# bioinformatics-centre/kaiju

Measured on NVIDIA H100. Metric: reads/sec (150 bp paired, MEM mode, synth-viruses .fmi), higher is better.
Workload: dtype int64

## Files before the change

### include/kaiju_b200.h

```cpp
#ifndef KAIJU_B200_H
#define KAIJU_B200_H
#include <stdint.h>

#ifdef __cplusplus
extern "C" {
#endif

typedef enum {
    KJ_OK = 0,
    KJ_ERR_ARG = -1,
    KJ_ERR_IO = -2,
    KJ_ERR_CUDA = -3,
    KJ_ERR_NO_DEVICE = -4,
    KJ_ERR_UNSUPPORTED = -5,
    KJ_ERR_OVERFLOW = -6,
    KJ_ERR_NOMEM = -7
} kj_status;

#define KJ_MAX_READ_LEN 16383
#define KJ_MAX_PROTEIN_LEN 5461
#define KJ_MAX_LONG_READ_LEN 1048575

typedef struct {
    int32_t mode;
// ... 102 lines not shown
    int32_t min_read_count;
    int32_t expand_viruses;
    int32_t filter_unclassified;
    int32_t full_path;
    const char *rank_list;
} kj_table_opts;
int kj_table_write(const uint64_t *taxon_ids, const uint64_t *counts, uint64_t n, const char *nodes_dmp, const char *names_dmp,
                   const char *label, const kj_table_opts *opts, const char *out_path, int append);
int kj_counts_table(kj_ctx *ctx, const char *nodes_dmp, const char *names_dmp, const char *label, const kj_table_opts *opts,
                    const char *out_path, int append);

int kj_check_errors(kj_ctx *ctx);

const char *kj_last_error(void);
uint64_t kj_kernel_launches(const kj_ctx *ctx);
uint64_t kj_index_bytes(const kj_ctx *ctx);
uint64_t kj_index_host_bytes(const kj_ctx *ctx);
int kj_index_layout(const kj_ctx *ctx);
double kj_last_kernel_ms(const kj_ctx *ctx);
int kj_launch_geometry(const kj_ctx *ctx, int *grid, int *block, int *dyn_smem_bytes);
int kj_version(void);
int kj_debug_index_checksums(kj_ctx *ctx, uint64_t out[8]);
int kj_debug_host_index_checksums(const kj_index_view *index, const kj_taxonomy_view *taxonomy, uint64_t out[8]);
int kj_debug_inflate_bgzf(kj_ctx *ctx, const uint8_t *file_bytes, uint64_t n, uint8_t *out, uint64_t out_cap, uint64_t *out_n,
                          uint64_t *first_bad_offset);

#ifdef __cplusplus
}
#endif
#endif
```

### kaiju_b200/__init__.py

```python
import ctypes as C
import os
import numpy as np

_HERE = os.path.dirname(os.path.abspath(__file__))
LIB_PATH = os.environ.get("KJ_B200_LIB") or os.path.join(_HERE, "libkaijub200.so")
MAX_READ_LEN = 16383
MAX_LONG_READ_LEN = 1048575

MEM, GREEDY = 0, 1
OUT_KAIJU, OUT_KAIJU_IDS, OUT_KAIJU_V, OUT_NAMES, OUT_NAMES_V = 0, 1, 2, 3, 4
STR_ACCESSION, STR_TAXON = 0, 1


class KjParams(C.Structure):
    _fields_ = [("mode", C.c_int32), ("min_fragment_length", C.c_uint32), ("mismatches", C.c_uint32),
                ("min_score", C.c_uint32), ("seed_length", C.c_uint32), ("use_evalue", C.c_int32),
                ("min_evalue", C.c_double), ("seg", C.c_int32), ("input_is_protein", C.c_int32), ("name_mode", C.c_int32)]


class KjIndexView(C.Structure):
    _fields_ = [("alen", C.c_int32), ("alphabet", C.c_char_p), ("bwtlen", C.c_int64), ("bwt", C.c_void_p),
                ("startLcode", C.c_void_p), ("db_len", C.c_int64), ("nseq", C.c_int32), ("ncheck", C.c_int64),
                ("chpt_exp", C.c_int32), ("nbytes", C.c_int32), ("pbits", C.c_int32), ("sa", C.c_void_p),
                ("seq_taxon", C.c_void_p), ("seq_accession", C.c_void_p)]
# ... 15 lines not shown
_lib = None


def lib():
    global _lib
    if _lib is None:
        if not os.path.exists(LIB_PATH):
            raise KaijuError("kaiju_b200: %s is missing -- build it with `make -C kaiju_b200/csrc` "
                             "(or python -c 'import __graft_entry__ as g; g.build()'). There is no CPU fallback." % LIB_PATH)
        L = C.CDLL(LIB_PATH)
        L.kj_last_error.restype = C.c_char_p
        L.kj_fmi_load.argtypes = [C.c_char_p, C.POINTER(C.c_void_p)]
        L.kj_fmi_view.argtypes = [C.c_void_p, C.POINTER(KjIndexView)]
        L.kj_fmi_free.argtypes = [C.c_void_p]
        L.kj_nodes_load.argtypes = [C.c_char_p, C.POINTER(C.c_void_p)]
        L.kj_nodes_view.argtypes = [C.c_void_p, C.POINTER(KjTaxonomyView)]
        L.kj_nodes_free.argtypes = [C.c_void_p]
        L.kj_create.argtypes = [C.POINTER(C.c_void_p), C.c_int, C.POINTER(KjParams), C.POINTER(KjIndexView), C.POINTER(KjTaxonomyView)]
        if hasattr(L, "kj_create_scaled"):
            L.kj_create_scaled.argtypes = [C.POINTER(C.c_void_p), C.c_int, C.POINTER(KjParams), C.POINTER(KjIndexView), C.POINTER(KjTaxonomyView), C.c_uint32]
            L.kj_index_build_ms.restype = C.c_double; L.kj_index_build_ms.argtypes = [C.c_void_p]
            L.kj_debug_index_checksums.argtypes = [C.c_void_p, C.c_void_p]
            L.kj_debug_host_index_checksums.argtypes = [C.POINTER(KjIndexView), C.POINTER(KjTaxonomyView), C.c_void_p]
            L.kj_classify_multi.argtypes = [C.POINTER(C.c_void_p), C.c_int, C.c_void_p, C.c_void_p, C.c_void_p, C.c_void_p, C.c_uint64, C.c_void_p, C.c_void_p]
            L.kj_device_count.restype = C.c_int
            L.kj_classify2.argtypes = [C.c_void_p, C.c_void_p, C.c_void_p, C.c_void_p, C.c_void_p, C.c_uint64, C.c_void_p, C.c_void_p, C.c_void_p]
            L.kj_classify_device2.argtypes = [C.c_void_p, C.c_void_p, C.c_void_p, C.c_void_p, C.c_void_p, C.c_uint64, C.c_uint32, C.c_uint32,
                                              C.c_void_p, C.c_void_p, C.c_void_p, C.c_void_p]
        L.kj_native_index_write.argtypes = [C.POINTER(KjIndexView), C.POINTER(KjTaxonomyView), C.c_char_p]
        L.kj_create_from_native.argtypes = [C.POINTER(C.c_void_p), C.c_int, C.POINTER(KjParams), C.c_char_p]
        L.kj_set_params.argtypes = [C.c_void_p, C.POINTER(KjParams)]
        L.kj_set_max_read_len.argtypes = [C.c_void_p, C.c_uint32]
        L.kj_destroy.argtypes = [C.c_void_p]
        L.kj_classify.argtypes = [C.c_void_p, C.c_void_p, C.c_void_p, C.c_void_p, C.c_void_p, C.c_uint64, C.c_void_p, C.c_void_p]
        L.kj_classify_verbose.argtypes = [C.c_void_p, C.c_void_p, C.c_void_p, C.c_void_p, C.c_void_p, C.c_uint64, C.c_void_p, C.c_void_p, C.c_void_p, C.c_void_p]
        L.kj_classify_device.argtypes = [C.c_void_p, C.c_void_p, C.c_void_p, C.c_void_p, C.c_void_p, C.c_uint64, C.c_uint32, C.c_uint32,
                                         C.c_void_p, C.c_void_p, C.c_void_p]
        L.kj_kernel_launches.restype = C.c_uint64; L.kj_kernel_launches.argtypes = [C.c_void_p]
        L.kj_index_bytes.restype = C.c_uint64; L.kj_index_bytes.argtypes = [C.c_void_p]
        if hasattr(L, "kj_create_tiered"):
            L.kj_create_tiered.argtypes = [C.POINTER(C.c_void_p), C.c_int, C.POINTER(KjParams), C.POINTER(KjIndexView), C.POINTER(KjTaxonomyView), C.c_uint32, C.c_uint64]
            L.kj_index_host_bytes.restype = C.c_uint64; L.kj_index_host_bytes.argtypes = [C.c_void_p]
        if hasattr(L, "kj_create_group"):
            L.kj_create_group.argtypes = [C.POINTER(C.c_void_p), C.c_int, C.POINTER(C.c_int), C.POINTER(KjParams), C.POINTER(KjIndexView), C.POINTER(KjTaxonomyView), C.c_uint32]
        if hasattr(L, "kj_index_layout"):
            L.kj_index_layout.restype = C.c_int; L.kj_index_layout.argtypes = [C.c_void_p]
# ... 291 lines not shown
    @property
    def kernel_launches(self):
        return int(lib().kj_kernel_launches(self._ctx))

    @property
    def index_bytes(self):
        return int(lib().kj_index_bytes(self._ctx))

    @property
    def layout(self):
        return int(lib().kj_index_layout(self._ctx))

    @property
    def host_bytes(self):
        return int(lib().kj_index_host_bytes(self._ctx))

    @property
    def index_build_ms(self):
        return float(lib().kj_index_build_ms(self._ctx))

    def debug_index_checksums(self):
        out = np.zeros(8, dtype=np.uint64); _check(lib().kj_debug_index_checksums(self._ctx, out.ctypes.data)); return out

    @property
    def last_kernel_ms(self):
        return float(lib().kj_last_kernel_ms(self._ctx))

    @property
    def launch_geometry(self):
        g = C.c_int(); b = C.c_int(); s = C.c_int()
        lib().kj_launch_geometry(self._ctx, C.byref(g), C.byref(b), C.byref(s))
        return g.value, b.value, s.value
```

### kaiju_b200/csrc/kj_build.h

```cpp
#pragma once

#define KJ_BLD_THREADS 256
struct KjBuildLcode { uint8_t v[256]; };

template <int RB>
__global__ void __launch_bounds__(KJ_BLD_THREADS) kj_bld_count(const uint8_t* __restrict__ bwt, const __grid_constant__ KjBuildLcode lc, uint64_t n, uint32_t rep, int alen,
                                                                uint32_t* __restrict__ tile_counts) {
    __shared__ uint32_t tot[KJ_MAX_ALEN];
    __shared__ uint8_t lcs[256];
    __shared__ uint8_t cnt[KJ_MAX_ALEN * KJ_BLD_THREADS];
    if (threadIdx.x < KJ_MAX_ALEN) tot[threadIdx.x] = 0;
    lcs[threadIdx.x] = lc.v[threadIdx.x];
    for (int a = 0; a < KJ_MAX_ALEN; a++) cnt[a * KJ_BLD_THREADS + threadIdx.x] = 0;
    __syncthreads();
    const uint64_t tile_rows = (uint64_t)KJ_BLD_THREADS * RB, start = (uint64_t)blockIdx.x * tile_rows;
    for (uint32_t i = threadIdx.x; i < tile_rows; i += KJ_BLD_THREADS) {
        const uint64_t row = start + i;
        if (row < n) cnt[(uint32_t)lcs[bwt[rep == 1 ? row : row / rep]] * KJ_BLD_THREADS + threadIdx.x]++;
    }
    for (int a = 0; a < alen; a++) {
        uint32_t v = cnt[a * KJ_BLD_THREADS + threadIdx.x];
        for (int m = 16; m > 0; m >>= 1) v += __shfl_xor_sync(0xffffffffu, v, m);
        if ((threadIdx.x & 31) == 0 && v) atomicAdd(&tot[a], v);
    }
// ... 74 lines not shown
        letters[wd] = v;
    }
}
__global__ void kj_bld_sa_tax(const uint8_t* __restrict__ sa, uint64_t n_entries, uint64_t first, int nbytes, int pbits, uint32_t nseq, const uint32_t* __restrict__ seq_tax,
                              uint32_t* __restrict__ sa_tax, uint32_t* __restrict__ err) {
    for (uint64_t e = (uint64_t)blockIdx.x * blockDim.x + threadIdx.x; e < n_entries; e += (uint64_t)gridDim.x * blockDim.x) {
        const uint8_t* p = sa + e * (uint64_t)nbytes; uint64_t val = 0;
        for (int b = 0; b < nbytes; b++) val = (val << 8) + p[b];
        const uint64_t seq = val >> pbits;
        if (seq >= nseq) { atomicOr(err, 64u); continue; }
        sa_tax[first + e] = seq_tax[seq];
    }
}
template <class IdxT>
__global__ void kj_bld_sa_tax_scaled(const KjDevIndex* __restrict__ base_ix, uint64_t n_entries, int64_t bias, int exp, uint64_t n_rows, uint32_t rep, uint32_t* __restrict__ sa_tax) {
    for (uint64_t e = (uint64_t)blockIdx.x * blockDim.x + threadIdx.x; e < n_entries; e += (uint64_t)gridDim.x * blockDim.x) {
        const uint64_t k = (uint64_t)((int64_t)e + bias) << exp;
        sa_tax[e] = k < n_rows ? kj_sa_taxon<IdxT>(*base_ix, k / rep) : KJ_TAX_BAD;
    }
}
__global__ void kj_bld_row_tax(const KjDevIndex* __restrict__ ix, uint64_t n_rows, uint32_t* __restrict__ row_tax) {
    for (uint64_t k = (uint64_t)blockIdx.x * blockDim.x + threadIdx.x; k < n_rows; k += (uint64_t)gridDim.x * blockDim.x) row_tax[k] = kj_row_taxon<uint32_t>(*ix, k);
}
__global__ void kj_bld_repeat_u32(const uint32_t* __restrict__ src, uint64_t n_out, uint32_t rep, uint32_t* __restrict__ dst) {
    for (uint64_t i = (uint64_t)blockIdx.x * blockDim.x + threadIdx.x; i < n_out; i += (uint64_t)gridDim.x * blockDim.x) dst[i] = src[i / rep];
}
template <class IdxT>
static __device__ __forceinline__ uint64_t kj_bld_rank(const KjDevIndex& ix, uint32_t c, uint64_t k) {
    uint64_t v = (uint64_t)kj_rank<IdxT>(ix, c, (IdxT)k);
    if (k >= ix.quirk_lo) v -= ix.quirk_d[c];
    return v;
}
template <class IdxT>
__global__ void kj_bld_quirk(const KjDevIndex* __restrict__ ix, uint64_t k, uint64_t* __restrict__ quirk_d) {
    const uint32_t a = threadIdx.x;
    if (a < (uint32_t)ix->alen) quirk_d[a] = (uint64_t)kj_rank<IdxT>(*ix, a, (IdxT)k) - ix->C[a];
}
template <class IdxT>
__global__ void kj_bld_kmer_level(const KjDevIndex* __restrict__ ix, const KjKmer* __restrict__ cur, uint64_t n_cur, KjKmer* __restrict__ nxt) {
    for (uint64_t t = (uint64_t)blockIdx.x * blockDim.x + threadIdx.x; t < n_cur * 20u; t += (uint64_t)gridDim.x * blockDim.x) {
        const KjKmer iv = cur[t / 20u]; const uint32_t a = (uint32_t)(t % 20u); KjKmer o; o.lo = 0; o.hi = 0;
        if (iv.lo < iv.hi) { o.lo = kj_bld_rank<IdxT>(*ix, a + 1u, iv.lo); o.hi = kj_bld_rank<IdxT>(*ix, a + 1u, iv.hi); if (o.lo >= o.hi) { o.lo = 0; o.hi = 0; } }
        nxt[t] = o;
    }
}
__global__ void kj_bld_kmer_narrow(const KjKmer* __restrict__ src, uint64_t n, KjKmer32* __restrict__ dst) {
// ... 348 lines not shown
    else {
        if ((rc = dst.grow(n_final * sizeof(KjKmer32)))) return rc;
        tot += n_final * sizeof(KjKmer32);
        kj_bld_kmer_narrow<<<c->sm_count * 8, 256>>>(a.as<KjKmer>(), n_final, dst.as<KjKmer32>()); CK(cudaGetLastError()); c->launches++;
    }
    CK(cudaDeviceSynchronize());
    k_out = k;
    return KJ_OK;
}

#define KJ_ROW_TAX_MARGIN (8ull << 30)
static int kj_device_build_row_tax(kj_ctx* c, uint64_t& tot) {
    const KjHostIndex& H = c->H;
    if (H.wide || kj_transient_ctx) return KJ_OK;
    const size_t bytes = (size_t)H.bwtlen * 4;
    size_t fr = 0, to = 0; CK(cudaMemGetInfo(&fr, &to));
    if (bytes + KJ_ROW_TAX_MARGIN > fr) return KJ_OK;
    int rc = c->row_tax.grow(bytes); if (rc) return rc;
    kj_bld_row_tax<<<c->sm_count * 16, 256>>>(c->ix.as<KjDevIndex>(), H.bwtlen, c->row_tax.as<uint32_t>());
    CK(cudaGetLastError()); CK(cudaDeviceSynchronize()); c->launches++;
    tot += bytes;
    return KJ_OK;
}
```

### kaiju_b200/csrc/kj_core.h

```cpp
#pragma once
#include "kj_warp.h"
#include "kj_layout.h"

#define KJ_SEG_CAP(max_frag) ((max_frag) / 4u + 8u)
struct KjKept { uint64_t lo; uint32_t len; uint32_t aux; };

template <bool LONG> struct KjW { typedef uint32_t pay; typedef uint16_t pos; };
template <> struct KjW<true> { typedef uint64_t pay; typedef uint32_t pos; };
#define KJ_LONG_LO_BITS 40

struct KjSmemLayout {
    uint32_t qkey_off, qpay_off, kept_off, res_off, res2_off, pre_off, ids_off, qord_off, aa_off, aa_stride, frag_off, hflag_off,
             segcnt_off, seghist_off, accs_off, total, segs_off;
#if defined(KJ_EMU)
    uint32_t guard[16], nguard;
#endif
};
#if defined(KJ_EMU)
#define KJ_GUARD(L, o) { (L).guard[(L).nguard++] = (o); (o) += 64u; }
#else
#define KJ_GUARD(L, o)
#endif
static KJ_HD uint32_t kj_align(uint32_t x, uint32_t a) { return (x + a - 1) / a * a; }
template <bool LONG = false>
// ... 217 lines not shown
template <class IdxT> struct KjChain { IdxT lo, hi; int i; int st; };

template <class IdxT>
static KJ_DEV void kj_chain_start(const KjDevIndex& ix, const uint8_t* frag, int j, uint32_t Lmin, KjChain<IdxT>& ch) {
    const int k = ix.kmer_k; int i = j; int budget = KJ_PHASE_A_LETTERS - 1;
    ch.st = KJ_ST_OPEN;
    if (k > 0 && j >= k && Lmin >= (uint32_t)k) {
        uint32_t idx = 0;
        KJ_ROLLED
        for (int t = 0; t < k; t++) idx = idx * 20u + (uint32_t)(frag[j - t] - 1u);
        IdxT lo, hi;
        if (sizeof(IdxT) == 4) { const KjKmer32 e = ((const KjKmer32*)ix.kmer)[idx]; lo = (IdxT)e.lo; hi = (IdxT)e.hi; }
        else { const KjKmer e = ((const KjKmer*)ix.kmer)[idx]; lo = (IdxT)e.lo; hi = (IdxT)e.hi; }
        if (lo >= hi) { ch.lo = 0; ch.hi = 0; ch.i = j + 1; ch.st = KJ_ST_KDEAD; return; }
        ch.lo = lo; ch.hi = hi; i = j - k + 1; budget = KJ_PHASE_A_LETTERS - k;
    } else {
        const uint32_t c = frag[j]; ch.lo = (IdxT)ix.C[c]; ch.hi = (IdxT)ix.C[c + 1];
    }
    KJ_ROLLED
    while (i > 0 && budget > 0) { if (!kj_update_si<IdxT>(ix, frag[i - 1], ch.lo, ch.hi)) { ch.st = KJ_ST_EXACT; break; } i--; budget--; }
    if (i == 0) ch.st = KJ_ST_EXACT;
    ch.i = i;
}
template <class IdxT>
static KJ_DEV void kj_chain_finish(const KjDevIndex& ix, const uint8_t* frag, KjChain<IdxT>& ch) {
    int i = ch.i;
    KJ_ROLLED
    while (i > 0) { if (!kj_update_si<IdxT>(ix, frag[i - 1], ch.lo, ch.hi)) break; i--; }
    ch.i = i; ch.st = KJ_ST_EXACT;
}
template <class IdxT>
static KJ_DEV void kj_finish_selected(const Warp& w, const KjDevIndex& ix, const uint8_t* frag, bool sel, KjChain<IdxT>& ch) {
#if defined(KJ_EMU)
    const int i0 = ch.i;
#endif
    if (sel) kj_chain_finish<IdxT>(ix, frag, ch);
    w.sync();
#if defined(KJ_EMU)
    { const uint32_t st = sel ? (uint32_t)(i0 - ch.i) + 1u : 0u; const uint32_t mx = warp_max_u32(w, st); const uint32_t nsel = (uint32_t)kj_popc(w.ballot(sel));
      uint32_t sum = st; for (int m = 16; m > 0; m >>= 1) sum += w.shfl_xor(sum, m);
      if (w.lane == 0) { kj_emu_stats.rounds++; kj_emu_stats.round_steps += mx; kj_emu_stats.lane_steps += sum; kj_emu_stats.chains += nsel; } }
#endif
}

template <class IdxT>
static KJ_DEV int kj_chain_lbval(const KjChain<IdxT>& ch, int j, int kk) { return ch.st == KJ_ST_EXACT ? ch.i : (j - kk + 2 > 0 ? j - kk + 2 : 0); }
template <class IdxT>
static KJ_DEV int kj_chain_lb(const Warp& w, const KjChain<IdxT>& ch, bool ran, int j, int kk, int lb_ext) {
    const uint32_t inf = w.ballot(ran && ch.st != KJ_ST_OPEN);
    const uint32_t below = w.lane < 31 ? inf & ~((2u << w.lane) - 1u) : 0u;
    const int v = w.shfl(kj_chain_lbval<IdxT>(ch, j, kk), below ? kj_ffs(below) - 1 : 0);
    return below ? v : lb_ext;
}
template <class IdxT>
static KJ_DEV int kj_block_lb_ext(const Warp& w, const KjChain<IdxT>& ch, bool ran, int j, int kk) {
    const uint32_t inf = w.ballot(ran && ch.st != KJ_ST_OPEN);
    const int v = w.shfl(kj_chain_lbval<IdxT>(ch, j, kk), inf ? kj_ffs(inf) - 1 : 0);
    return inf ? v : 0;
}
static KJ_DEV uint32_t kj_prefix_max_excl(const Warp& w, uint32_t v, uint32_t init) {
    for (int d = 1; d < 32; d <<= 1) { const uint32_t o = w.shfl(v, w.lane - d); if (w.lane >= d && o > v) v = o; }
    const uint32_t e = w.shfl(v, w.lane - 1);
// ... 708 lines not shown
            const bool open = act && cur.st == KJ_ST_OPEN && w.lane <= cut;
            const uint32_t om = w.ballot(open);
            uint32_t nm = 0; bool need = false;
            if (om) {
                int lb = 0;
                if (mono) {
                    int lb_ext = 0;
                    if (round > 0 && !have_nxt && jhi - 32 >= 0) {
                        const uint32_t inf = w.ballot(act && cur.st != KJ_ST_OPEN);
                        if ((31 - kj_clz(om)) > (inf ? 31 - kj_clz(inf) : -1)) { jstart = jhi - 32; start_la = true; continue; }
                    }
                    if (have_nxt) lb_ext = kj_block_lb_ext<IdxT>(w, nxt, jhi - 32 - w.lane >= 0, jhi - 32 - w.lane, kk);
                    lb = kj_chain_lb<IdxT>(w, cur, act, j, kk, lb_ext);
                }
                const uint32_t exl = (act && cur.st == KJ_ST_EXACT && w.lane <= cut) ? (uint32_t)(j - cur.i + 1) : 0u;
                const uint32_t Lb = kj_prefix_max_excl(w, exl, L);
                need = open && j >= (int)Lb - 1 && !(lb >= 2 && (uint32_t)(j - lb + 1) < Lb);
                nm = w.ballot(need);
            }
            if (nm) {
                const bool top = need && !(w.lane > 0 && ((nm >> (w.lane - 1)) & 1u));
                const int group = (round == 0 && mono) ? 0 : KJ_GROUP_LATE;
                const bool sel = need && (top || kj_popc(nm & lanemask_lt(w.lane)) < group);
                kj_finish_selected<IdxT>(w, ix, frag, sel, cur);
                round++;
                continue;
            }
            const bool valid = act && w.lane <= cut;
            const uint32_t l = (valid && cur.st == KJ_ST_EXACT) ? (uint32_t)(j - cur.i + 1) : 0u;
            const uint32_t lmax = warp_max_u32(w, l);
            if (lmax >= L) {
                if (lmax > item_best) { item_best = lmax; item_cnt = 0; }
                L = lmax;
                const uint32_t wm = w.ballot(l == item_best && l > 0);
                if (l == item_best && l > 0) { KjKept* k = kj_kept_ptr(cx, nkept + item_cnt + (uint32_t)kj_popc(wm & lanemask_lt(w.lane))); k->lo = (uint64_t)cur.lo; k->len = (uint32_t)(cur.hi - cur.lo);
                                               k->aux = LONG ? (arr << 29) | (start + 3u * (uint32_t)cur.i) : (arr << 29) | ((start + 3u * (uint32_t)cur.i) << 14) | l; }
                item_cnt += (uint32_t)kj_popc(wm);
            }
            jhi -= 32;
            if (brk || jhi < (int)L - 1) break;
            round = 0;
            if (have_nxt) { cur = nxt; have_nxt = false; } else { jstart = jhi; start_la = false; }
        }
        w.sync();
        if (item_cnt > 0 && rp.seg && !segchecked && kj_seg_gate<LONG>(cx, q, arr, start, len, false)) return true;
        if (item_cnt > 0) {
            const uint32_t keep = rp.name_mode ? 1u : 0u;
// ... 143 lines not shown
```

### kaiju_b200/csrc/kj_core_greedy.h

```cpp
#pragma once
#include "kj_core.h"

template <bool LONG = false>
struct alignas(16) KjVariant {
    uint64_t lo, hi;
    typename KjW<LONG>::pay pay;
    int32_t diff;
    typename KjW<LONG>::pos matchlen; uint8_t num_mm; uint8_t pad;
    uint32_t subs[KJ_MAX_MM];
    uint32_t pad2;
};
static_assert(sizeof(KjVariant<>) == 64, "KjVariant is one 64-byte record");
template <bool LONG = false>
static KJ_HD uint32_t kj_greedy_scratch_bytes(const KjRunParams& rp) { return rp.mode == 1 ? rp.variant_cap * (uint32_t)(sizeof(KjVariant<LONG>) + 8u) : 64u; }

template <bool LONG = false>
struct KjMatch { uint64_t lo; uint32_t len; typename KjW<LONG>::pos qi, ql; };
static_assert(sizeof(KjMatch<false>) == 16 && sizeof(KjMatch<true>) == 24, "kj_smem_layout sizes the result arrays with these");

template <bool LONG = false>
struct KjVQueue { uint64_t* gkey; KjVariant<LONG>* v; uint32_t n, live;
    KJ_DEV uint64_t& key(uint32_t s) const { return gkey[s]; } };

template <class V>
// ... 88 lines not shown
        kj_load_frag(cx, arr, start, len);
        if ((uint32_t)w.lane < nsub) frag[mysub >> 5] = (uint8_t)(mysub & 31u);
        w.sync();
        if (rp.seg && !segchecked && kj_seg_gate<LONG>(cx, q, arr, start, len, true)) continue;

        {
            uint32_t carry = 0;
            KJ_ROLLED
            for (uint32_t b = 0; b < len; b += 32) {
                uint32_t t = b + (uint32_t)w.lane; uint32_t a = t < len ? frag[t] : 0u;
                uint32_t d = t < len ? (uint32_t)tb.b62[a][a] : 0u;
                uint32_t sc = kj_scan_incl(w, d) + carry;
                if (t < len) pre[t + 1] = (PosT)sc;
                carry = w.shfl(sc, 31);
            }
            if (w.lane == 0) pre[0] = 0;
            w.sync();
        }

        uint32_t nrec = 0;
        if (num_mm > 0) {
            KjChain<IdxT> one; one.lo = (IdxT)si0; one.hi = (IdxT)si1; one.i = (int)len - (int)matchlen; one.st = KJ_ST_OPEN;
#if defined(KJ_EMU)
            const int i0_ = one.i;
#endif
            kj_chain_finish<IdxT>(ix, frag, one);
#if defined(KJ_EMU)
            if (w.lane == 0) kj_emu_stats.var_steps += (unsigned long long)(i0_ - one.i + 1);
#endif
            const IdxT lo = one.lo, hi = one.hi; const int i = one.i;
            uint32_t l = len - (uint32_t)i;
            uint32_t Lreq = (num_mm == rp.e) ? rp.m : matchlen;
            if (l >= Lreq) { if (w.lane == 0) { cls[0].lo = (uint64_t)lo; cls[0].len = (uint32_t)(hi - lo); cls[0].qi = (PosT)i; cls[0].ql = (PosT)l; } nrec = 1; }
            w.sync();
        } else {
            const int L = (int)rp.seed_length;
            const bool mono = ix.mono != 0; const int kk = ix.kmer_k;
            int jlow = (int)len; uint32_t qi_above = 0xffffffffu;
            int jhi = (int)len - 1, jstart = jhi, round = 0; bool start_la = false, have_nxt = false;
            KjChain<IdxT> cur, nxt;
            cur.lo = 0; cur.hi = 0; cur.i = 0; cur.st = KJ_ST_EXACT; nxt = cur;
            KJ_ROLLED
            for (;;) {
                if (jstart >= 0) {
                    KjChain<IdxT> t; t.lo = 0; t.hi = 0; t.i = 0; t.st = KJ_ST_EXACT;
                    if (jstart - w.lane >= L - 1 || (start_la && jstart - w.lane >= 0)) kj_chain_start<IdxT>(ix, frag, jstart - w.lane, rp.seed_length, t);
                    w.sync();
                    if (start_la) { nxt = t; have_nxt = true; } else { cur = t; round = 0; }
                    jstart = -1;
                }
                const int j = jhi - w.lane; const bool act = j >= L - 1;
// ... 236 lines not shown
```

### kaiju_b200/csrc/kj_device.cu

```cuda
#include <cuda_runtime.h>
#include <algorithm>
#include <chrono>
#include <cmath>
#include <cstdio>
#include <cstdlib>
#include <cstring>
#include <map>
#include <memory>
#include <mutex>
#include <string>
#include <thread>
#include <vector>
#include "kj_core.h"
#include "kj_core_greedy.h"
#include "kj_host.h"

#define KJ_WARPS_PER_CTA 8
#define KJ_MIN_BLOCKS 4
#define KJ_MIN_BLOCKS_GREEDY_SPLIT 4
#define KJ_MIN_BLOCKS_GREEDY 4
#define KJ_CLAIM 4
#define KJ_CHUNK_READS (1u << 20)
#define KJ_CHUNK_BYTES (1ull << 28)
#define KJ_LONG_GAP 4096u
// ... 224 lines not shown

struct KjSlot {
    KjDevBuf seq[2], off[2];
    KjDevBuf tax, best, ids, nids, acc, nacc, frag, fraglen;
    KjDevBuf spill, gscratch, ws;
    bool long_scratch = false;
    cudaStream_t stream = nullptr, fstream = nullptr;
    cudaEvent_t ev_in = nullptr, ev_f[2] = {nullptr, nullptr}, ev_s[2] = {nullptr, nullptr};
};

struct KjFilesState; static void kj_files_state_free(KjFilesState* S);
struct kj_ctx {
    std::unique_ptr<KjFilesState, void (*)(KjFilesState*)> files{nullptr, kj_files_state_free};
    int device = 0; kj_params params{}; int sm_count = 0;
    KjHostIndex H;
    KjDevIndex dix{};
    KjDevBuf ix, tables;
    KjDevBuf ix_mem, kmer_mem; int kmer_k_mem = 0;
    KjDevBuf rank, letters, tax_parent, tax_depth, tax_id, lnfact, kmer;
    KjTierBuf sa_tax, seq_tax, sa_acc, seq_acc;
    KjHostBuf rank_host; uint64_t nb_dev = 0;
    std::shared_ptr<KjGroup> group;
    KjDevBuf row_tax;
    KjTierBuf out_str[2], out_off[2]; uint64_t out_n[2] = {0, 0}, out_bytes[2] = {0, 0}; bool out_have[2] = {false, false};
    uint64_t index_bytes = 0, host_bytes = 0; uint64_t n_sa = 0; double build_ms = 0.0;
    KjDevBuf counter, err, maxlen, quirk;
    KjDevBuf evbreaks; uint32_t n_evbreaks = 0;
    KjDevBuf counts, counts_pending; uint32_t n_counts = 0, n_present = 0;
    uint32_t variant_boost = 1;
    uint32_t max_read_len = KJ_MAX_READ_LEN;
    KjDevBuf prep;
    KjSlot slot[2];
    cudaEvent_t ev_a = nullptr, ev_b = nullptr;
    uint64_t launches = 0; double last_kernel_ms = 0.0;
    int grid = 0; size_t smem_bytes = 0; KjKernel grid_kernel = nullptr;
};

struct KjOut {
    uint64_t* tax = nullptr; uint32_t* best = nullptr; uint32_t* compact = nullptr;
    uint64_t* ids = nullptr; uint8_t* nids = nullptr;
    uint32_t* acc = nullptr; uint8_t* nacc = nullptr;
    char* frag = nullptr; uint32_t frag_stride = 0; uint32_t* fraglen = nullptr;
    unsigned long long* counts = nullptr;
};

template <class T> static int upload(const std::vector<T>& v, KjDevBuf& d, uint64_t& total) {
// ... 54 lines not shown
    if (device < 0 || device >= ndev) { kj_err() = "device ordinal out of range"; return KJ_ERR_ARG; }
    CK(cudaSetDevice(device));
    kj_ctx* c = new kj_ctx(); c->device = device; c->params = *params;
    std::unique_ptr<kj_ctx, void (*)(kj_ctx*)> guard(c, kj_destroy);
    cudaDeviceProp prop; CK(cudaGetDeviceProperties(&prop, device)); c->sm_count = prop.multiProcessorCount;
    if ((rc = c->err.grow(sizeof(uint32_t)))) return rc;
    CK(cudaMemset(c->err.p, 0, sizeof(uint32_t)));
    if ((rc = c->quirk.grow(sizeof c->H.quirk_d))) return rc;
    CK(cudaMemset(c->quirk.p, 0, sizeof c->H.quirk_d));
    *out = guard.release(); return KJ_OK;
}
static int upload_descriptor(kj_ctx* c) {
    KjHostIndex& H = c->H; KjDevIndex& D = c->dix; memset(&D, 0, sizeof D);
    D.rank = c->rank.as<const uint64_t>(); D.nb = H.nb; D.letters = c->letters.as<const uint64_t>(); D.bwtlen = H.bwtlen; D.alen = H.alen;
    for (int a = 0; a <= H.alen; a++) D.C[a] = H.C[a];
    if (!kj_is_compact(H.wide)) for (int a = 0; a < H.alen; a++) D.rank_base[a] = D.rank + (uint64_t)a * H.nb * kj_rank_words(H.wide);
    if (H.wide == KJ_LAYOUT_COMPACT_TIERED) { D.tier.host = c->rank_host.as<const uint64_t>(); D.tier.nb_dev = c->nb_dev; }
    const KjGroup* G = c->group.get();
    if (H.wide == KJ_LAYOUT_COMPACT_SPREAD) { D.spread = G->ref; D.rank = G->ref.base[0]; }
    const KjTierBuf& sa_acc = G ? G->sa_acc : c->sa_acc; const KjTierBuf& seq_acc = G ? G->seq_acc : c->seq_acc;
    const KjTierBuf& sa_tax = G ? G->sa_tax : c->sa_tax; const KjTierBuf& seq_tax = G ? G->seq_tax : c->seq_tax;
    D.sa_acc = sa_acc.as<const uint32_t>(); D.seq_acc = seq_acc.as<const uint32_t>();
    D.sa_tax = sa_tax.as<const uint32_t>(); D.seq_tax = seq_tax.as<const uint32_t>(); D.sa_check = H.sa_check; D.sa_exp = H.sa_exp; D.sa_bias = H.sa_bias;
    D.n_sa = c->n_sa; D.row_tax = c->row_tax.as<const uint32_t>(); D.nseq = H.nseq;
    D.tax_parent = c->tax_parent.as<const uint32_t>(); D.tax_depth = c->tax_depth.as<const uint32_t>(); D.tax_id = c->tax_id.as<const uint64_t>(); D.n_tax = (uint32_t)H.tax_id.size();
    D.lnfact = c->lnfact.as<const double>(); D.n_lnfact = (int)H.lnfact.size(); D.kmer = H.kmer_k ? c->kmer.p : nullptr; D.kmer_k = H.kmer_k; D.wide = H.wide; D.tables = c->tables.as<KjTables>();
    D.quirk_lo = H.quirk_lo; D.mono = H.quirk_lo == ~0ull ? 1 : 0; D.quirk_d = c->quirk.as<uint64_t>();
    int rc = c->ix.grow(sizeof(KjDevIndex)); if (rc) return rc;
    CK(cudaMemcpy(c->ix.p, &D, sizeof(KjDevIndex), cudaMemcpyHostToDevice));
    if (c->kmer_mem.p && c->kmer_k_mem) {
        KjDevIndex M = D; M.kmer = c->kmer_mem.p; M.kmer_k = c->kmer_k_mem;
        if ((rc = c->ix_mem.grow(sizeof(KjDevIndex)))) return rc;
        CK(cudaMemcpy(c->ix_mem.p, &M, sizeof(KjDevIndex), cudaMemcpyHostToDevice));
    }
    return KJ_OK;
}
static int upload_small(kj_ctx* c, uint64_t& tot) {
    KjHostIndex& H = c->H; int rc;
    if ((rc = upload(H.tax_parent, c->tax_parent, tot)) || (rc = upload(H.tax_depth, c->tax_depth, tot)) || (rc = upload(H.tax_id, c->tax_id, tot)) || (rc = upload(H.lnfact, c->lnfact, tot)) ||
        (rc = c->tables.grow(sizeof(KjTables)))) return rc;
    CK(cudaMemcpy(c->tables.p, &H.tables, sizeof(KjTables), cudaMemcpyHostToDevice));
    return KJ_OK;
}
static int kj_device_build_row_tax(kj_ctx* c, uint64_t& tot);
static int finish_ctx(kj_ctx* c, uint64_t tot) {
    KjHostIndex& H = c->H; int rc;
    CK(cudaMemcpy(c->quirk.p, H.quirk_d, sizeof H.quirk_d, cudaMemcpyHostToDevice));
    if ((rc = upload_descriptor(c)) || (rc = kj_device_build_row_tax(c, tot)) || (rc = upload_descriptor(c))) return rc;
    c->index_bytes = tot;
    if ((rc = c->counter.grow(4 * sizeof(unsigned long long))) || (rc = c->maxlen.grow(2 * sizeof(unsigned int)))) return rc;
    for (KjSlot& S : c->slot) {
        CK(cudaStreamCreateWithFlags(&S.stream, cudaStreamNonBlocking)); CK(cudaStreamCreateWithFlags(&S.fstream, cudaStreamNonBlocking));
        CK(cudaEventCreateWithFlags(&S.ev_in, cudaEventDisableTiming));
        for (int b = 0; b < 2; b++) { CK(cudaEventCreateWithFlags(&S.ev_f[b], cudaEventDisableTiming)); CK(cudaEventCreateWithFlags(&S.ev_s[b], cudaEventDisableTiming)); }
    }
    CK(cudaEventCreate(&c->ev_a)); CK(cudaEventCreate(&c->ev_b));
    if ((rc = upload_evalue_breaks(c))) return rc;
    c->n_counts = (uint32_t)H.tax_id.size() + 1u; c->n_present = H.n_present;
    if ((rc = c->counts.grow((size_t)c->n_counts * 8)) || (rc = c->counts_pending.grow((size_t)c->n_counts * 8))) return rc;
    CK(cudaMemset(c->counts.p, 0, (size_t)c->n_counts * 8)); CK(cudaMemset(c->counts_pending.p, 0, (size_t)c->n_counts * 8));
    return KJ_OK;
}

template <class Fill> static int create_ctx(kj_ctx** out, int device, const kj_params* params, Fill fill) {
    kj_ctx* c = nullptr; int rc = new_ctx(&c, device, params); if (rc) return rc;
    std::unique_ptr<kj_ctx, void (*)(kj_ctx*)> guard(c, kj_destroy);
    rc = fill(c->H); if (rc) return rc;
    KjHostIndex& H = c->H; uint64_t tot = 0;
    c->n_sa = H.sa_tax.size(); H.sa_tax.push_back(KJ_TAX_BAD);
    if (!H.seq_acc.empty()) { H.sa_acc.push_back(0xffffffffu); if ((rc = tier_upload(c, H.sa_acc, c->sa_acc, tot)) || (rc = tier_upload(c, H.seq_acc, c->seq_acc, tot))) return rc; }
    if ((rc = upload(H.rank, c->rank, tot)) || (rc = upload(H.letters, c->letters, tot)) || (rc = tier_upload(c, H.sa_tax, c->sa_tax, tot)) ||
// ... 104 lines not shown
        }
        if ((rc = finish_ctx(c, ct))) return rc;
    }
    for (int g = 0; g < n; g++) {
        kj_ctx* c = raw[g]; c->index_bytes += G->seg[g].cap;
        if (std::find(devices, devices + g, c->device) != devices + g) continue;
        for (const KjTierBuf* b : {&G->sa_tax, &G->seq_tax, &G->sa_acc, &G->seq_acc}) if (b->p && b->device == c->device) c->index_bytes += b->cap();
    }
    for (kj_ctx* c : raw) { CK(cudaSetDevice(c->device)); CK(cudaDeviceSynchronize()); }
    const double ms = std::chrono::duration<double, std::milli>(std::chrono::steady_clock::now() - t0).count();
    for (int g = 0; g < n; g++) { raw[g]->build_ms = ms; out[g] = cs[g].release(); }
    return KJ_OK;
}
extern "C" int kj_create_group(kj_ctx** out, int n, const int* devices, const kj_params* params, const kj_index_view* index, const kj_taxonomy_view* taxonomy, uint32_t copies) {
    if (!out || !devices || !params || !index || !taxonomy) { kj_err() = "kj_create_group: null argument"; return KJ_ERR_ARG; }
    if (n < 1 || n > KJ_MAX_GROUP) { kj_err() = "kj_create_group: a group has 1 to " + std::to_string(KJ_MAX_GROUP) + " devices, not " + std::to_string(n); return KJ_ERR_ARG; }
    const int ndev = kj_device_count();
    for (int g = 0; g < n; g++)
        if (ndev > 0 && (devices[g] < 0 || devices[g] >= ndev)) { kj_err() = "kj_create_group: device ordinal " + std::to_string(devices[g]) + " out of range"; return KJ_ERR_ARG; }
    for (int g = 0; g < n; g++) out[g] = nullptr;
    return create_group_device(out, n, devices, params, *index, *taxonomy, copies < 1 ? 1 : copies);
}
extern "C" double kj_index_build_ms(const kj_ctx* c) { return c ? c->build_ms : 0.0; }
extern "C" int kj_debug_index_checksums(kj_ctx* c, uint64_t out[8]) {
    if (!c || !out) return KJ_ERR_ARG; CK(cudaSetDevice(c->device)); CK(cudaDeviceSynchronize());
    const KjHostIndex& H = c->H; memset(out, 0, 64);
    const size_t sz[5] = {(size_t)kj_rank_array_words(H.wide, H.alen, H.nb) * 8, (size_t)kj_letters_words(H.wide, H.bwtlen) * 8, (size_t)c->n_sa * 4, (size_t)H.nseq * 4,
                          H.kmer_k ? (size_t)pow(20.0, H.kmer_k) * (H.wide ? sizeof(KjKmer) : sizeof(KjKmer32)) : 0};
    const KjGroup* G = c->group.get();
    const void* ptr[5] = {c->rank.p, c->letters.p, G ? G->sa_tax.p : c->sa_tax.p, G ? G->seq_tax.p : c->seq_tax.p, c->kmer.p};
    const size_t dev0 = H.wide == KJ_LAYOUT_COMPACT_TIERED ? (size_t)c->nb_dev * KJ_RANK_WORDS_COMPACT * 8 : G ? 0 : sz[0];
    for (int i = 0; i < 5; i++) {
        std::vector<uint8_t> h(sz[i]); const size_t nd = i == 0 ? dev0 : sz[i];
        if (nd) CK(cudaMemcpy(h.data(), ptr[i], nd, cudaMemcpyDefault));
        if (i == 0 && G) {
            for (int g = 0; g < G->n; g++) {
                const size_t o = (size_t)G->first[g] * KJ_RANK_WORDS_COMPACT * 8, b = (size_t)(G->first[g + 1] - G->first[g]) * KJ_RANK_WORDS_COMPACT * 8;
                if (b) CK(cudaMemcpy(h.data() + o, G->seg[g].p, b, cudaMemcpyDefault));
            }
        } else if (i == 0 && sz[0] > dev0) memcpy(h.data() + dev0, c->rank_host.p, sz[0] - dev0);
        out[i] = kj_mix_bytes(0x6b616a75ull + i, h.data(), h.size());
    }
    out[5] = H.bwtlen; out[6] = (uint64_t)H.wide; out[7] = c->n_sa;
    return KJ_OK;
}

// ... 386 lines not shown
```

### kaiju_b200/csrc/kj_layout.h

```cpp
#pragma once
#include <stddef.h>
#include <stdint.h>

#define KJ_LAYOUT_NARROW 0
#define KJ_LAYOUT_WIDE 1
#define KJ_LAYOUT_COMPACT 2
#define KJ_LAYOUT_COMPACT_TIERED 3
#define KJ_LAYOUT_COMPACT_SPREAD 4
#define KJ_MAX_GROUP 8
#define KJ_RANK_ROWS_NARROW 64
#define KJ_RANK_ROWS_WIDE 192
#define KJ_RANK_ROWS_COMPACT 128
#define KJ_RANK_WORDS_NARROW 2
#define KJ_RANK_WORDS_WIDE 4
#define KJ_RANK_WORDS_COMPACT 16
#define KJ_CPT_COUNT_WORD 10
#define KJ_CSB_SHIFT 16
#define KJ_CSB_STRIDE 24
static inline bool kj_is_compact(int layout) { return layout == KJ_LAYOUT_COMPACT || layout == KJ_LAYOUT_COMPACT_TIERED || layout == KJ_LAYOUT_COMPACT_SPREAD; }
static inline uint32_t kj_rank_rows(int layout) { return kj_is_compact(layout) ? KJ_RANK_ROWS_COMPACT : layout ? KJ_RANK_ROWS_WIDE : KJ_RANK_ROWS_NARROW; }
static inline uint32_t kj_rank_words(int layout) { return kj_is_compact(layout) ? KJ_RANK_WORDS_COMPACT : layout ? KJ_RANK_WORDS_WIDE : KJ_RANK_WORDS_NARROW; }
static inline uint64_t kj_rank_array_words(int layout, int alen, uint64_t nb) { return (kj_is_compact(layout) ? 1ull : (uint64_t)alen) * nb * kj_rank_words(layout); }
static inline uint64_t kj_csb_count(uint64_t bwtlen) { return (bwtlen >> KJ_CSB_SHIFT) + 1; }
#define KJ_LETTERS_PER_WORD 12
// ... 29 lines not shown
    const uint64_t* rank; uint64_t nb;
    union {
        const uint64_t* rank_base[KJ_MAX_ALEN];
        KjTierRef tier;
        KjSpreadRef spread;
    };
    union {
        const uint64_t* letters;
        const uint64_t* csb;
    };
    uint64_t bwtlen; int alen; uint32_t nseq;
    uint64_t C[KJ_MAX_ALEN + 1];
    const uint32_t* sa_tax; const uint32_t* seq_tax;
    const uint32_t* sa_acc; const uint32_t* seq_acc;
    uint64_t sa_check; int sa_exp; int64_t sa_bias; uint64_t n_sa;
    const uint32_t* row_tax;
    const uint32_t* tax_parent; const uint32_t* tax_depth; const uint64_t* tax_id; uint32_t n_tax; int n_lnfact;
    const double* lnfact;
    const void* kmer; int kmer_k;
    int wide;
    int mono;
    uint64_t quirk_lo; const uint64_t* quirk_d;
    const KjTables* tables;
};
static_assert(sizeof(KjTierRef) <= sizeof(const uint64_t*) * KJ_MAX_ALEN && sizeof(KjDevIndex) == 592 && offsetof(KjDevIndex, rank_base) == 16 &&
              offsetof(KjDevIndex, tier) == 16 && offsetof(KjDevIndex, letters) == 208 && offsetof(KjDevIndex, tables) == 584, "KjDevIndex layout changed");
static_assert(sizeof(KjSpreadRef) == 136 && sizeof(KjSpreadRef) <= sizeof(const uint64_t*) * KJ_MAX_ALEN && offsetof(KjDevIndex, spread) == 16,
              "the segment table must fit in rank_base's bytes");

struct KjRunParams {
    int mode;
    uint32_t m, e, min_score, seed_length;
    int use_evalue, seg, protein, name_mode;
    const double* ev_breaks; uint32_t n_ev_breaks;
    uint32_t max_len;
    uint32_t max_frag;
    uint32_t item_cap;
    uint32_t kept_cap_smem;
    uint32_t scratch_entries;
    uint32_t variant_cap;
    uint32_t ws_global;
};
```

Before: 57.09 million.

## Precompute six-step LF jump table for singleton intervals in MEM chain extension

Builds a per-row table on the device storing the next six BWT letters and the row reached after six LF steps. During MEM backward extension, when the SA interval has width one, the code checks the next six query letters against the stored letters and jumps six steps with a single load instead of six rank lookups. This spends bwtlen*8 bytes of device memory and build time, and adds branching and divergence inside the warp loop. Mismatching jumps fall back to single-step extension.

```diff
diff --git a/include/kaiju_b200.h b/include/kaiju_b200.h
--- a/include/kaiju_b200.h
+++ b/include/kaiju_b200.h
@@ -148,6 +148,7 @@
 int kj_version(void);
 int kj_debug_index_checksums(kj_ctx *ctx, uint64_t out[8]);
 int kj_debug_host_index_checksums(const kj_index_view *index, const kj_taxonomy_view *taxonomy, uint64_t out[8]);
+int kj_debug_lf6(kj_ctx *ctx, uint64_t *out, uint64_t cap, uint64_t *n);
 int kj_debug_inflate_bgzf(kj_ctx *ctx, const uint8_t *file_bytes, uint64_t n, uint8_t *out, uint64_t out_cap, uint64_t *out_n,
                           uint64_t *first_bad_offset);
 
diff --git a/kaiju_b200/__init__.py b/kaiju_b200/__init__.py
--- a/kaiju_b200/__init__.py
+++ b/kaiju_b200/__init__.py
@@ -61,6 +61,7 @@
             L.kj_index_build_ms.restype = C.c_double; L.kj_index_build_ms.argtypes = [C.c_void_p]
             L.kj_debug_index_checksums.argtypes = [C.c_void_p, C.c_void_p]
             L.kj_debug_host_index_checksums.argtypes = [C.POINTER(KjIndexView), C.POINTER(KjTaxonomyView), C.c_void_p]
+            L.kj_debug_lf6.argtypes = [C.c_void_p, C.c_void_p, C.c_uint64, C.POINTER(C.c_uint64)]
             L.kj_classify_multi.argtypes = [C.POINTER(C.c_void_p), C.c_int, C.c_void_p, C.c_void_p, C.c_void_p, C.c_void_p, C.c_uint64, C.c_void_p, C.c_void_p]
             L.kj_device_count.restype = C.c_int
             L.kj_classify2.argtypes = [C.c_void_p, C.c_void_p, C.c_void_p, C.c_void_p, C.c_void_p, C.c_uint64, C.c_void_p, C.c_void_p, C.c_void_p]
@@ -398,6 +399,12 @@
     def debug_index_checksums(self):
         out = np.zeros(8, dtype=np.uint64); _check(lib().kj_debug_index_checksums(self._ctx, out.ctypes.data)); return out
 
+    def debug_lf6(self):
+        n = C.c_uint64(0); _check(lib().kj_debug_lf6(self._ctx, None, 0, C.byref(n)))
+        if n.value == 0:
+            return None
+        out = np.zeros(n.value, dtype=np.uint64); _check(lib().kj_debug_lf6(self._ctx, out.ctypes.data, n.value, C.byref(n))); return out
+
     @property
     def last_kernel_ms(self):
         return float(lib().kj_last_kernel_ms(self._ctx))
diff --git a/kaiju_b200/csrc/kj_build.h b/kaiju_b200/csrc/kj_build.h
--- a/kaiju_b200/csrc/kj_build.h
+++ b/kaiju_b200/csrc/kj_build.h
@@ -120,6 +120,9 @@
 __global__ void kj_bld_row_tax(const KjDevIndex* __restrict__ ix, uint64_t n_rows, uint32_t* __restrict__ row_tax) {
     for (uint64_t k = (uint64_t)blockIdx.x * blockDim.x + threadIdx.x; k < n_rows; k += (uint64_t)gridDim.x * blockDim.x) row_tax[k] = kj_row_taxon<uint32_t>(*ix, k);
 }
+__global__ void kj_bld_lf6(const KjDevIndex* __restrict__ ix, uint64_t n_rows, uint64_t* __restrict__ lf6) {
+    for (uint64_t k = (uint64_t)blockIdx.x * blockDim.x + threadIdx.x; k < n_rows; k += (uint64_t)gridDim.x * blockDim.x) lf6[k] = kj_lf6_entry(*ix, (uint32_t)k);
+}
 __global__ void kj_bld_repeat_u32(const uint32_t* __restrict__ src, uint64_t n_out, uint32_t rep, uint32_t* __restrict__ dst) {
     for (uint64_t i = (uint64_t)blockIdx.x * blockDim.x + threadIdx.x; i < n_out; i += (uint64_t)gridDim.x * blockDim.x) dst[i] = src[i / rep];
 }
@@ -514,3 +517,15 @@
     tot += bytes;
     return KJ_OK;
 }
+static int kj_device_build_lf6(kj_ctx* c, uint64_t& tot) {
+    const KjHostIndex& H = c->H;
+    if (H.wide || kj_transient_ctx) return KJ_OK;
+    const size_t bytes = (size_t)H.bwtlen * 8;
+    size_t fr = 0, to = 0; CK(cudaMemGetInfo(&fr, &to));
+    if (bytes + KJ_ROW_TAX_MARGIN > fr) return KJ_OK;
+    int rc = c->lf6.grow(bytes); if (rc) return rc;
+    kj_bld_lf6<<<c->sm_count * 16, 256>>>(c->ix.as<KjDevIndex>(), H.bwtlen, c->lf6.as<uint64_t>());
+    CK(cudaGetLastError()); CK(cudaDeviceSynchronize()); c->launches++;
+    tot += bytes;
+    return KJ_OK;
+}
diff --git a/kaiju_b200/csrc/kj_core.h b/kaiju_b200/csrc/kj_core.h
--- a/kaiju_b200/csrc/kj_core.h
+++ b/kaiju_b200/csrc/kj_core.h
@@ -263,22 +263,68 @@
     if (i == 0) ch.st = KJ_ST_EXACT;
     ch.i = i;
 }
-template <class IdxT>
-static KJ_DEV void kj_chain_finish(const KjDevIndex& ix, const uint8_t* frag, KjChain<IdxT>& ch) {
-    int i = ch.i;
-    KJ_ROLLED
-    while (i > 0) { if (!kj_update_si<IdxT>(ix, frag[i - 1], ch.lo, ch.hi)) break; i--; }
+#define KJ_LF6_STEP 6
+static KJ_DEV uint64_t kj_lf6_entry(const KjDevIndex& ix, uint32_t k) {
+    uint64_t letters = 0;
+    KJ_ROLLED
+    for (int t = 0; t < KJ_LF6_STEP; t++) {
+        const uint32_t c = kj_letter(ix, k);
+        if (c == 0) break;
+        letters |= (uint64_t)c << (5 * t);
+        k = kj_rank<uint32_t>(ix, c, k);
+    }
+    return letters << 32 | k;
+}
+template <class IdxT, bool JUMP = false>
+static KJ_DEV int kj_chain_finish(const KjDevIndex& ix, const uint8_t* frag, KjChain<IdxT>& ch) {
+    int i = ch.i, trips = 0;
+    if constexpr (JUMP && sizeof(IdxT) == 4) {
+        const uint64_t* lf6 = ix.lf6;
+        if (lf6) {
+            int stop = 0;
+            KJ_ROLLED
+            while (i > stop) {
+                const uint32_t lo = (uint32_t)ch.lo, hi = (uint32_t)ch.hi, c = frag[i - 1];
+                const bool jump = stop == 0 && i >= KJ_LF6_STEP && hi - lo == 1u;
+                const uint64_t* base = kj_letter_base(ix, c);
+                const uint64_t* p0 = jump ? lf6 + (lo & ~1u) : base + 2u * (size_t)(lo >> 6);
+                uint64_t h0, w0, h1, w1;
+                kj_ld128(p0, h0, w0); kj_ld128(base + 2u * (size_t)(hi >> 6), h1, w1);
+                trips++;
+                if (jump) {
+                    uint32_t want = 0;
+                    #pragma unroll
+                    for (int t = 0; t < KJ_LF6_STEP; t++) want |= (uint32_t)frag[i - 1 - t] << (5 * t);
+                    const uint64_t e = (lo & 1u) ? w0 : h0;
+                    const uint32_t x = (uint32_t)(e >> 32) ^ want;
+                    if (x == 0) { ch.lo = (IdxT)(uint32_t)e; ch.hi = ch.lo + 1u; i -= KJ_LF6_STEP; }
+                    else stop = i - (int)((uint32_t)(kj_ffs(x) - 1) / 5u);
+                    continue;
+                }
+                const uint32_t nlo = (uint32_t)h0 + (uint32_t)kj_popcll(w0 & ((1ull << (lo & 63u)) - 1ull));
+                const uint32_t nhi = (uint32_t)h1 + (uint32_t)kj_popcll(w1 & ((1ull << (hi & 63u)) - 1ull));
+                if (nlo >= nhi) break;
+                ch.lo = (IdxT)nlo; ch.hi = (IdxT)nhi; i--;
+            }
+            ch.i = i; ch.st = KJ_ST_EXACT;
+            return trips;
+        }
+    }
+    KJ_ROLLED
+    while (i > 0) { trips++; if (!kj_update_si<IdxT>(ix, frag[i - 1], ch.lo, ch.hi)) break; i--; }
     ch.i = i; ch.st = KJ_ST_EXACT;
-}
-template <class IdxT>
+    return trips;
+}
+template <class IdxT, bool JUMP = false>
 static KJ_DEV void kj_finish_selected(const Warp& w, const KjDevIndex& ix, const uint8_t* frag, bool sel, KjChain<IdxT>& ch) {
 #if defined(KJ_EMU)
-    const int i0 = ch.i;
-#endif
-    if (sel) kj_chain_finish<IdxT>(ix, frag, ch);
+    const int trips = sel ? kj_chain_finish<IdxT, JUMP>(ix, frag, ch) : 0;
+#else
+    if (sel) kj_chain_finish<IdxT, JUMP>(ix, frag, ch);
+#endif
     w.sync();
 #if defined(KJ_EMU)
-    { const uint32_t st = sel ? (uint32_t)(i0 - ch.i) + 1u : 0u; const uint32_t mx = warp_max_u32(w, st); const uint32_t nsel = (uint32_t)kj_popc(w.ballot(sel));
+    { const uint32_t st = (uint32_t)trips; const uint32_t mx = warp_max_u32(w, st); const uint32_t nsel = (uint32_t)kj_popc(w.ballot(sel));
       uint32_t sum = st; for (int m = 16; m > 0; m >>= 1) sum += w.shfl_xor(sum, m);
       if (w.lane == 0) { kj_emu_stats.rounds++; kj_emu_stats.round_steps += mx; kj_emu_stats.lane_steps += sum; kj_emu_stats.chains += nsel; } }
 #endif
@@ -1033,7 +1079,7 @@
                 const bool top = need && !(w.lane > 0 && ((nm >> (w.lane - 1)) & 1u));
                 const int group = (round == 0 && mono) ? 0 : KJ_GROUP_LATE;
                 const bool sel = need && (top || kj_popc(nm & lanemask_lt(w.lane)) < group);
-                kj_finish_selected<IdxT>(w, ix, frag, sel, cur);
+                kj_finish_selected<IdxT, true>(w, ix, frag, sel, cur);
                 round++;
                 continue;
             }
diff --git a/kaiju_b200/csrc/kj_core_greedy.h b/kaiju_b200/csrc/kj_core_greedy.h
--- a/kaiju_b200/csrc/kj_core_greedy.h
+++ b/kaiju_b200/csrc/kj_core_greedy.h
@@ -134,11 +134,10 @@
         if (num_mm > 0) {
             KjChain<IdxT> one; one.lo = (IdxT)si0; one.hi = (IdxT)si1; one.i = (int)len - (int)matchlen; one.st = KJ_ST_OPEN;
 #if defined(KJ_EMU)
-            const int i0_ = one.i;
-#endif
+            const int trips_ = kj_chain_finish<IdxT>(ix, frag, one);
+            if (w.lane == 0) kj_emu_stats.var_steps += (unsigned long long)trips_;
+#else
             kj_chain_finish<IdxT>(ix, frag, one);
-#if defined(KJ_EMU)
-            if (w.lane == 0) kj_emu_stats.var_steps += (unsigned long long)(i0_ - one.i + 1);
 #endif
             const IdxT lo = one.lo, hi = one.hi; const int i = one.i;
             uint32_t l = len - (uint32_t)i;
diff --git a/kaiju_b200/csrc/kj_device.cu b/kaiju_b200/csrc/kj_device.cu
--- a/kaiju_b200/csrc/kj_device.cu
+++ b/kaiju_b200/csrc/kj_device.cu
@@ -270,6 +270,7 @@
     KjHostBuf rank_host; uint64_t nb_dev = 0;
     std::shared_ptr<KjGroup> group;
     KjDevBuf row_tax;
+    KjDevBuf lf6;
     KjTierBuf out_str[2], out_off[2]; uint64_t out_n[2] = {0, 0}, out_bytes[2] = {0, 0}; bool out_have[2] = {false, false};
     uint64_t index_bytes = 0, host_bytes = 0; uint64_t n_sa = 0; double build_ms = 0.0;
     KjDevBuf counter, err, maxlen, quirk;
@@ -370,7 +371,7 @@
     const KjTierBuf& sa_tax = G ? G->sa_tax : c->sa_tax; const KjTierBuf& seq_tax = G ? G->seq_tax : c->seq_tax;
     D.sa_acc = sa_acc.as<const uint32_t>(); D.seq_acc = seq_acc.as<const uint32_t>();
     D.sa_tax = sa_tax.as<const uint32_t>(); D.seq_tax = seq_tax.as<const uint32_t>(); D.sa_check = H.sa_check; D.sa_exp = H.sa_exp; D.sa_bias = H.sa_bias;
-    D.n_sa = c->n_sa; D.row_tax = c->row_tax.as<const uint32_t>(); D.nseq = H.nseq;
+    D.n_sa = c->n_sa; D.row_tax = c->row_tax.as<const uint32_t>(); D.lf6 = c->lf6.as<const uint64_t>(); D.nseq = H.nseq;
     D.tax_parent = c->tax_parent.as<const uint32_t>(); D.tax_depth = c->tax_depth.as<const uint32_t>(); D.tax_id = c->tax_id.as<const uint64_t>(); D.n_tax = (uint32_t)H.tax_id.size();
     D.lnfact = c->lnfact.as<const double>(); D.n_lnfact = (int)H.lnfact.size(); D.kmer = H.kmer_k ? c->kmer.p : nullptr; D.kmer_k = H.kmer_k; D.wide = H.wide; D.tables = c->tables.as<KjTables>();
     D.quirk_lo = H.quirk_lo; D.mono = H.quirk_lo == ~0ull ? 1 : 0; D.quirk_d = c->quirk.as<uint64_t>();
@@ -391,10 +392,11 @@
     return KJ_OK;
 }
 static int kj_device_build_row_tax(kj_ctx* c, uint64_t& tot);
+static int kj_device_build_lf6(kj_ctx* c, uint64_t& tot);
 static int finish_ctx(kj_ctx* c, uint64_t tot) {
     KjHostIndex& H = c->H; int rc;
     CK(cudaMemcpy(c->quirk.p, H.quirk_d, sizeof H.quirk_d, cudaMemcpyHostToDevice));
-    if ((rc = upload_descriptor(c)) || (rc = kj_device_build_row_tax(c, tot)) || (rc = upload_descriptor(c))) return rc;
+    if ((rc = upload_descriptor(c)) || (rc = kj_device_build_row_tax(c, tot)) || (rc = kj_device_build_lf6(c, tot)) || (rc = upload_descriptor(c))) return rc;
     c->index_bytes = tot;
     if ((rc = c->counter.grow(4 * sizeof(unsigned long long))) || (rc = c->maxlen.grow(2 * sizeof(unsigned int)))) return rc;
     for (KjSlot& S : c->slot) {
@@ -545,6 +547,12 @@
     return create_group_device(out, n, devices, params, *index, *taxonomy, copies < 1 ? 1 : copies);
 }
 extern "C" double kj_index_build_ms(const kj_ctx* c) { return c ? c->build_ms : 0.0; }
+extern "C" int kj_debug_lf6(kj_ctx* c, uint64_t* out, uint64_t cap, uint64_t* n) {
+    if (!c || !n || (cap && !out)) return KJ_ERR_ARG; CK(cudaSetDevice(c->device)); CK(cudaDeviceSynchronize());
+    *n = c->lf6.p ? c->H.bwtlen : 0;
+    if (*n && cap) CK(cudaMemcpy(out, c->lf6.p, (size_t)std::min(cap, *n) * 8, cudaMemcpyDeviceToHost));
+    return KJ_OK;
+}
 extern "C" int kj_debug_index_checksums(kj_ctx* c, uint64_t out[8]) {
     if (!c || !out) return KJ_ERR_ARG; CK(cudaSetDevice(c->device)); CK(cudaDeviceSynchronize());
     const KjHostIndex& H = c->H; memset(out, 0, 64);
diff --git a/kaiju_b200/csrc/kj_layout.h b/kaiju_b200/csrc/kj_layout.h
--- a/kaiju_b200/csrc/kj_layout.h
+++ b/kaiju_b200/csrc/kj_layout.h
@@ -75,8 +75,9 @@
     int mono;
     uint64_t quirk_lo; const uint64_t* quirk_d;
     const KjTables* tables;
+    const uint64_t* lf6;
 };
-static_assert(sizeof(KjTierRef) <= sizeof(const uint64_t*) * KJ_MAX_ALEN && sizeof(KjDevIndex) == 592 && offsetof(KjDevIndex, rank_base) == 16 &&
+static_assert(sizeof(KjTierRef) <= sizeof(const uint64_t*) * KJ_MAX_ALEN && sizeof(KjDevIndex) == 600 && offsetof(KjDevIndex, rank_base) == 16 &&
               offsetof(KjDevIndex, tier) == 16 && offsetof(KjDevIndex, letters) == 208 && offsetof(KjDevIndex, tables) == 584, "KjDevIndex layout changed");
 static_assert(sizeof(KjSpreadRef) == 136 && sizeof(KjSpreadRef) <= sizeof(const uint64_t*) * KJ_MAX_ALEN && offsetof(KjDevIndex, spread) == 16,
               "the segment table must fit in rank_base's bytes");
```

Measured after the change: 56.22 million, median of 6. 0.985x the previous value.
